# TimZaman/dotaclient

Hardware: NVIDIA H100
Metric: optimizer_steps_per_sec (higher is better)
Workload: dtype f32

## Files before the change

dotaclient_b200/csrc/dc_common.cuh:

```cuda
#pragma once
#include <cuda_runtime.h>
#include <stdint.h>
#include "dotaclient_b200.h"

void dc_set_error(const char *fmt, ...);

#define DC_REQUIRE(cond, code, ...)        \
    do {                                   \
        if (!(cond)) {                     \
            dc_set_error(__VA_ARGS__);     \
            return (code);                 \
        }                                  \
    } while (0)

#define DC_CUDA(call)                                                                      \
    do {                                                                                   \
        cudaError_t e__ = (call);                                                          \
        if (e__ != cudaSuccess) {                                                          \
            dc_set_error("%s failed at %s:%d: %s", #call, __FILE__, __LINE__,              \
                         cudaGetErrorString(e__));                                         \
            return (int)e__;                                                               \
        }                                                                                  \
    } while (0)

#define DC_LAUNCH_OK() DC_CUDA(cudaGetLastError())

static inline cudaStream_t dc_cu_stream(dc_stream_t s) { return reinterpret_cast<cudaStream_t>(s); }

int dc_sm_count();

int dc_gemm_tf32x3_splitk(const float *A, int lda, const float *B, int ldb, float *part, int64_t M, int N, int K, int ksplit,
                          bool first_call, cudaStream_t st);

int dc_unit_basic_reduce(const float *partial, int nblocks, float *dw_b, float *db_b, int accumulate, cudaStream_t st);

__device__ __forceinline__ float dc_sigmoid(float x) { return 1.0f / (1.0f + __expf(-x)); }
__device__ __forceinline__ float dc_tanh(float x) { return 1.0f - 2.0f / (__expf(2.0f * x) + 1.0f); }

__device__ __forceinline__ float2 dc_ffma2(float2 a, float2 b, float2 c) { return make_float2(fmaf(a.x, b.x, c.x), fmaf(a.y, b.y, c.y)); }

__device__ __forceinline__ uint32_t dc_smem_u32(const void *p) { return (uint32_t)__cvta_generic_to_shared(p); }
__device__ __forceinline__ float dc_tf32_rna(float v) { return __uint_as_float((__float_as_uint(v) + 0x1000u) & 0xffffe000u); }
__device__ __forceinline__ uint64_t dc_wgmma_desc(uint32_t smem_addr) {
    return (uint64_t)((smem_addr & 0x3FFFF) >> 4) | (1ull << 16) | ((uint64_t)(1024 >> 4) << 32) | (1ull << 62);
}
__device__ __forceinline__ void dc_wgmma_fence() { asm volatile("wgmma.fence.sync.aligned;" ::: "memory"); }
__device__ __forceinline__ void dc_wgmma_commit() { asm volatile("wgmma.commit_group.sync.aligned;" ::: "memory"); }
__device__ __forceinline__ void dc_wgmma_wait0() { asm volatile("wgmma.wait_group.sync.aligned 0;" ::: "memory"); }
__device__ __forceinline__ void dc_reg_fence(float &r) { asm volatile("" : "+f"(r)::"memory"); }
__device__ __forceinline__ void dc_mbar_init(uint64_t *bar, int count) {
    asm volatile("mbarrier.init.shared::cta.b64 [%0], %1;" ::"r"(dc_smem_u32(bar)), "r"(count));
}
__device__ __forceinline__ void dc_mbar_arrive(uint64_t *bar) {
    asm volatile("mbarrier.arrive.shared::cta.b64 _, [%0];" ::"r"(dc_smem_u32(bar)) : "memory");
}
__device__ __forceinline__ void dc_mbar_wait(uint64_t *bar, uint32_t parity) {
    uint32_t ok;
    do {
        asm volatile("{ .reg .pred p; mbarrier.try_wait.parity.shared::cta.b64 p, [%1], %2; selp.u32 %0, 1, 0, p; }"
                     : "=r"(ok)
                     : "r"(dc_smem_u32(bar)), "r"(parity)
                     : "memory");
    } while (!ok);
}

__device__ __forceinline__ float dc_warp_sum(float v) {
#pragma unroll
    for (int o = 16; o > 0; o >>= 1) v += __shfl_xor_sync(0xffffffffu, v, o);
    return v;
}
__device__ __forceinline__ double dc_warp_sum(double v) {
#pragma unroll
    for (int o = 16; o > 0; o >>= 1) v += __shfl_xor_sync(0xffffffffu, v, o);
    return v;
}
```

dotaclient_b200/csrc/gemm_tf32x3.cu:

```cuda
#include "dc_common.cuh"
#include "unit_basic.cuh"

namespace {

constexpr int BM = 128, BN = 128, BK = 32;
constexpr int kStages = 2;
constexpr int kTileBytes = BM * BK * 4;
constexpr int kStageBytes = 4 * kTileBytes;
constexpr int kProducerThreads = 128;
constexpr int kProducerGroups = kStages;
constexpr int kConsumerWarp0 = 4 * kProducerGroups;
constexpr int kConsumerThreads = 256;
constexpr int kThreads = kConsumerWarp0 * 32 + kConsumerThreads;
constexpr int kLdS = BN + 8;
constexpr int kDIn = kUnitFeatures;
constexpr size_t kOffStaging = (size_t)kStages * kStageBytes;
constexpr size_t kOffBars = kOffStaging + (size_t)BM * kLdS * 4;
constexpr size_t kSmemBytes = kOffBars + 128 + 1024 ;

#define DC_ACC8(b) "+f"(d[b]), "+f"(d[b + 1]), "+f"(d[b + 2]), "+f"(d[b + 3]), "+f"(d[b + 4]), "+f"(d[b + 5]), "+f"(d[b + 6]), "+f"(d[b + 7])
__device__ __forceinline__ void wgmma_m64n128k8(float (&d)[64], uint64_t desc_a, uint64_t desc_b) {
    asm volatile(
        "{\n\t.reg .pred p;\n\tsetp.ne.b32 p, %66, 0;\n\t"
        "wgmma.mma_async.sync.aligned.m64n128k8.f32.tf32.tf32 "
// ... 894 lines not shown
            const int t0 = (split + j * nsplit) * kRPC, tend = min(T, t0 + kRPC);
            const int s = j % kWgStages;
            dc_mbar_wait(&empty[s], ((j / kWgStages) & 1) ^ 1);
            unsigned char *st = ring + (size_t)s * kWgStageBytes;
            const uint32_t xs = dc_smem_u32(st + 2 * kTileBytes);
#pragma unroll
            for (int r = 0; r < BK / 4; ++r) {
                const int row = (t >> 5) + 4 * r;
                const bool ok = xc_in && t0 + row < tend;
                const size_t xr = kDevT && x_rows != nullptr && ok ? (size_t)__ldg(x_rows + t0 + row) : (size_t)(t0 + row);
                cp_async16(xs + (row * kWgLdX + 4 * xc) * 4, X + (ok ? xr * ldx + n0 + 4 * xc : 0), ok ? 16u : 0u);
            }
            cp_async_arrive(&full[s]);
            store_row_k(va, st, st + kTileBytes, t);
            asm volatile("fence.proxy.async.shared::cta;" ::: "memory");
            __syncwarp();
            if (lane == 0) dc_mbar_arrive(&full[s]);
        }
        colsum_s[g * 128 + t] = cs;
        asm volatile("cp.async.wait_all;" ::: "memory");
    } else {
        const int ct = threadIdx.x - kConsumerWarp0 * 32, wg = ct >> 7, w4 = (ct >> 5) & 3, q = lane & 3;
        const int rlo = 64 * wg + 16 * w4 + (lane >> 2);
        float d[64];
#pragma unroll
        for (int i = 0; i < 64; ++i) d[i] = 0.f;
        uint32_t ahi[2][4] = {}, alo[2][4] = {};
#pragma unroll
        for (int i = 0; i < 64; ++i) dc_reg_fence(d[i]);
        float *pt = part_w + ((size_t)split * tiles_mn + tile) * BM * BN + ct * 4;
        const auto flush = [&](bool add) {
            dc_wgmma_wait0();
#pragma unroll
            for (int k = 0; k < 64; ++k) dc_reg_fence(d[k]);
            if (add) {
#pragma unroll
                for (int m = 0; m < 16; ++m)
                    asm volatile("red.global.add.v4.f32 [%0], {%1, %2, %3, %4};" ::"l"(pt + m * kConsumerThreads * 4), "f"(d[4 * m]),
                                 "f"(d[4 * m + 1]), "f"(d[4 * m + 2]), "f"(d[4 * m + 3]) : "memory");
            } else {
#pragma unroll
                for (int m = 0; m < 16; ++m)
                    *reinterpret_cast<float4 *>(pt + m * kConsumerThreads * 4) = make_float4(d[4 * m], d[4 * m + 1], d[4 * m + 2], d[4 * m + 3]);
            }
#pragma unroll
            for (int k = 0; k < 64; ++k) d[k] = 0.f;
#pragma unroll
            for (int k = 0; k < 64; ++k) dc_reg_fence(d[k]);
        };
        int j = 0;
        do {
            const int j_end = min(my_chunks, j + kWgFlush);
            for (; j < j_end; ++j) {
                const int s = j % kWgStages;
                dc_mbar_wait(&full[s], (j / kWgStages) & 1);
                const uint32_t st = dc_smem_u32(ring + (size_t)s * kWgStageBytes);
                const uint32_t xk = st + 2 * kTileBytes + (q * kWgLdX + rlo) * 4;
                float v[16];
#pragma unroll
                for (int ks = 0; ks < BK / 8; ++ks) {
                    const uint32_t x8 = xk + 8 * ks * kWgLdX * 4;
                    v[4 * ks] = lds_f32(x8);
                    v[4 * ks + 1] = lds_f32(x8 + 8 * 4);
                    v[4 * ks + 2] = lds_f32(x8 + 4 * kWgLdX * 4);
                    v[4 * ks + 3] = lds_f32(x8 + (4 * kWgLdX + 8) * 4);
                }
                const uint64_t b_hi = dc_wgmma_desc(st), b_lo = dc_wgmma_desc(st + kTileBytes);
#pragma unroll
                for (int ks = 0; ks < BK / 8; ++ks) {
                    const int b = ks & 1;
#pragma unroll
                    for (int e = 0; e < 4; ++e) {
                        const float h = dc_tf32_rna(v[4 * ks + e]);
                        ahi[b][e] = __float_as_uint(h);
                        alo[b][e] = __float_as_uint(v[4 * ks + e] - h);
                    }
                    dc_wgmma_fence();
                    const uint64_t adv = (uint64_t)(ks * 2);
                    wgmma_m64n128k8_rs(d, ahi[b][0], ahi[b][1], ahi[b][2], ahi[b][3], b_lo + adv);
                    wgmma_m64n128k8_rs(d, alo[b][0], alo[b][1], alo[b][2], alo[b][3], b_hi + adv);
                    wgmma_m64n128k8_rs(d, ahi[b][0], ahi[b][1], ahi[b][2], ahi[b][3], b_hi + adv);
                    dc_wgmma_commit();
                    wgmma_wait1();
#pragma unroll
                    for (int e = 0; e < 4; ++e) asm volatile("" : "+r"(ahi[b ^ 1][e]), "+r"(alo[b ^ 1][e])::"memory");
                    if (ks == 0 && j > 0) {
                        __syncwarp();
                        if (lane == 0) dc_mbar_arrive(&empty[(j - 1) % kWgStages]);
                    }
                }
            }
            flush(j > kWgFlush);
        } while (j < my_chunks);
    }
    __syncthreads();
    if (part_b != nullptr && n0 == 0 && threadIdx.x < 128 && m0 + (int)threadIdx.x < No)
        part_b[(size_t)split * No + m0 + threadIdx.x] = colsum_s[threadIdx.x] + colsum_s[128 + threadIdx.x];
}

constexpr int kRedRows = 8;
__global__ void __launch_bounds__(32 * kRedRows) wgrad_reduce_kernel(const float *__restrict__ part_w, const float *__restrict__ part_b,
                                                                     int nsplit, int No, int Ni, float *__restrict__ dW, int ldw,
                                                                     float *__restrict__ db, int accumulate) {
    __shared__ float4 sh[kRedRows][32];
    const int x = threadIdx.x & 31, y = threadIdx.x >> 5;
    const int n_blocks = (Ni + BN - 1) / BN, tiles_mn = ((No + BM - 1) / BM) * n_blocks;
    const int total4 = tiles_mn * (BM * BN / 4), bias4 = db != nullptr ? No / 4 : 0;
    const int idx = blockIdx.x * 32 + x;
    const float *src = nullptr;
    size_t stride = 0;
    if (idx < total4) {
        src = part_w + (size_t)idx * 4;
        stride = (size_t)tiles_mn * BM * BN;
    } else if (idx < total4 + bias4) {
        src = part_b + (size_t)(idx - total4) * 4;
        stride = (size_t)No;
    }
    float4 acc = make_float4(0.f, 0.f, 0.f, 0.f);
    if (src != nullptr) {
#pragma unroll 4
        for (int s = y; s < nsplit; s += kRedRows) {
            const float4 v = __ldg(reinterpret_cast<const float4 *>(src + (size_t)s * stride));
            acc.x += v.x; acc.y += v.y; acc.z += v.z; acc.w += v.w;
        }
    }
    sh[y][x] = acc;
    __syncthreads();
    if (y == 0 && src != nullptr) {
        if (idx < total4) {
            const int tile = idx / (BM * BN / 4), r = idx % (BM * BN / 4), m = r / kConsumerThreads, ct = r % kConsumerThreads;
            const int o = (tile / n_blocks) * BM + 8 * m + 2 * (ct & 3);
            const int i = (tile % n_blocks) * BN + 64 * (ct >> 7) + 16 * ((ct >> 5) & 3) + ((ct & 31) >> 2);
            float *p[4];
            float v[4];
#pragma unroll
            for (int e = 0; e < 4; ++e) {
                const int oe = o + (e & 1), ie = i + 8 * (e >> 1);
                p[e] = oe < No && ie < Ni ? dW + (size_t)oe * ldw + ie : nullptr;
                v[e] = accumulate && p[e] != nullptr ? *p[e] : 0.f;
            }
#pragma unroll
            for (int r = 0; r < kRedRows; ++r) { v[0] += sh[r][x].x; v[1] += sh[r][x].y; v[2] += sh[r][x].z; v[3] += sh[r][x].w; }
#pragma unroll
            for (int e = 0; e < 4; ++e)
                if (p[e] != nullptr) *p[e] = v[e];
        } else {
            float *dst = db + (size_t)(idx - total4) * 4;
            float4 t = accumulate ? *reinterpret_cast<const float4 *>(dst) : make_float4(0.f, 0.f, 0.f, 0.f);
#pragma unroll
            for (int r = 0; r < kRedRows; ++r) { t.x += sh[r][x].x; t.y += sh[r][x].y; t.z += sh[r][x].z; t.w += sh[r][x].w; }
            *reinterpret_cast<float4 *>(dst) = t;
        }
    }
}

}

extern "C" int dc_gemm_tf32x3_supported(int64_t M, int N, int K) { return M > 0 && N > 0 && K > 0 && N % 32 == 0 && K % BK == 0; }

struct RowList {
    const int *count, *a_rows, *rows;
    float *C_rows;
};

template <int NU, bool kGenA = false, bool kDevM = false>
static int launch_ws(const float *A, int lda, const float *B, int ldb, const float *bias, float *C, int ldc, int M, int N,
                     int K, int relu, float *C_copy, uint8_t *argmax, cudaStream_t st, GenA gen = GenA{}, RowList rl = RowList{}) {
    const int tile_rows = NU == 5 ? 60 : kWsRows;
    const int n_blocks = (N + BN - 1) / BN, m_blocks = (M + tile_rows - 1) / tile_rows;
    int per_block = dc_sm_count() / n_blocks;
    if (per_block < 1) per_block = 1;
    if (per_block > m_blocks) per_block = m_blocks;
    const size_t smem = kGenA ? kWsGenSmemBytes : kWsSmemBytes;
    DC_CUDA(cudaFuncSetAttribute(gemm_ws_kernel<NU, kGenA, kDevM>, cudaFuncAttributeMaxDynamicSharedMemorySize, (int)smem));
    gemm_ws_kernel<NU, kGenA, kDevM><<<n_blocks * per_block, kWsThreads, smem, st>>>(A, lda, B, ldb, bias, C, ldc, M, N, K, relu, C_copy,
                                                                                    argmax, gen, rl.count, rl.a_rows, rl.rows, rl.C_rows);
    DC_LAUNCH_OK();
    return DC_OK;
}

static int gemm_check_shape(const float *A, int lda, const float *B, int ldb, const float *bias, const float *C, int ldc, int64_t M,
                            int N, int K, const char *who) {
    DC_REQUIRE(dc_gemm_tf32x3_supported(M, N, K) && M < (1ll << 31) - BM, DC_EUNSUPPORTED,
               "%s: need N %% 32 == 0 and K %% 32 == 0 (M=%lld N=%d K=%d)", who, (long long)M, N, K);
    DC_REQUIRE(lda >= K && ldb >= K && ldc >= N && lda % 4 == 0 && ldb % 4 == 0 && ldc % 4 == 0, DC_EINVAL,
               "%s: leading dimensions must be >= extent and multiples of 4 floats", who);
    DC_REQUIRE(((uintptr_t)A & 15) == 0 && ((uintptr_t)B & 15) == 0 && ((uintptr_t)C & 15) == 0 && (!bias || ((uintptr_t)bias & 15) == 0),
               DC_EINVAL, "%s: pointers must be 16-byte aligned", who);
    return DC_OK;
}

static int gemm_check(const float *A, int lda, const float *B, int ldb, const float *bias, const float *C, int ldc, int64_t M, int N,
                      int K, const char *who) {
    DC_REQUIRE(A && B && C, DC_EINVAL, "%s: null pointer", who);
    return gemm_check_shape(A, lda, B, ldb, bias, C, ldc, M, N, K, who);
}

template <bool kDevM>
static int gemm_launch(const float *A, int lda, const float *B, int ldb, const float *bias, float *C, int ldc, int64_t M, int N, int K,
                       int relu, RowList rl, cudaStream_t st) {
    if (K <= 4 * BK) return launch_ws<0, false, kDevM>(A, lda, B, ldb, bias, C, ldc, (int)M, N, K, relu, nullptr, nullptr, st, GenA{}, rl);
    const int tiles = (int)((M + BM - 1) / BM) * ((N + BN - 1) / BN);
    DC_CUDA(cudaFuncSetAttribute(gemm_tf32x3_kernel<kDevM>, cudaFuncAttributeMaxDynamicSharedMemorySize, (int)kSmemBytes));
    const int grid = tiles < dc_sm_count() ? tiles : dc_sm_count();
    gemm_tf32x3_kernel<kDevM><<<grid, kThreads, kSmemBytes, st>>>(A, lda, B, ldb, bias, C, ldc, (int)M, N, K, relu, 1, 0, rl.count,
                                                                  rl.a_rows, rl.rows, rl.C_rows);
    DC_LAUNCH_OK();
    return DC_OK;
}

extern "C" int dc_gemm_tf32x3(const float *A, int lda, const float *B, int ldb, const float *bias, float *C, int ldc,
                              int64_t M, int N, int K, int relu, dc_stream_t stream) {
    const int rc = gemm_check(A, lda, B, ldb, bias, C, ldc, M, N, K, "dc_gemm_tf32x3");
    if (rc != DC_OK) return rc;
    return gemm_launch<false>(A, lda, B, ldb, bias, C, ldc, M, N, K, relu, RowList{}, dc_cu_stream(stream));
}

extern "C" int dc_gemm_tf32x3_rows(const float *A, int lda, const float *B, int ldb, const float *bias, float *C, float *C_rows, int ldc,
                                   int64_t M, const int32_t *count, const int32_t *rows, int gather_a, int N, int K, int relu,
                                   dc_stream_t stream) {
    DC_REQUIRE(A && B && count && (C || C_rows) && (rows || (!gather_a && !C_rows)), DC_EINVAL, "dc_gemm_tf32x3_rows: null pointer");
    DC_REQUIRE(((uintptr_t)C_rows & 15) == 0, DC_EINVAL, "dc_gemm_tf32x3_rows: pointers must be 16-byte aligned");
    const int rc = gemm_check_shape(A, lda, B, ldb, bias, C, ldc, M, N, K, "dc_gemm_tf32x3_rows");
    if (rc != DC_OK) return rc;
    return gemm_launch<true>(A, lda, B, ldb, bias, C, ldc, M, N, K, relu, RowList{count, gather_a ? rows : nullptr, rows, C_rows},
                             dc_cu_stream(stream));
}

int dc_gemm_tf32x3_splitk(const float *A, int lda, const float *B, int ldb, float *part, int64_t M, int N, int K, int ksplit,
                          bool first_call, cudaStream_t st) {
    DC_REQUIRE(A && B && part && ksplit >= 1 && N % BN == 0 && K % (BK * ksplit) == 0 && M > 0, DC_EINVAL,
               "dc_gemm_tf32x3_splitk: bad arguments (M=%lld N=%d K=%d ksplit=%d)", (long long)M, N, K, ksplit);
    if (first_call)
        DC_CUDA(cudaFuncSetAttribute(gemm_tf32x3_kernel<false>, cudaFuncAttributeMaxDynamicSharedMemorySize, (int)kSmemBytes));
    const int tiles = (int)((M + BM - 1) / BM) * (N / BN) * ksplit;
    const int grid = tiles < dc_sm_count() ? tiles : dc_sm_count();
    gemm_tf32x3_kernel<false><<<grid, kThreads, kSmemBytes, st>>>(A, lda, B, ldb, nullptr, part, N, (int)M, N, K, 0, ksplit, (long long)M * N);
    DC_LAUNCH_OK();
    return DC_OK;
}

static int wgrad_tiles(int No, int Ni) { return ((No + BM - 1) / BM) * ((Ni + BN - 1) / BN); }

static int wgrad_splits(int No, int Ni) {
    const int tiles_mn = wgrad_tiles(No, Ni);
    const int n = dc_sm_count() / tiles_mn;
    return n < 1 ? 1 : n;
}

extern "C" size_t dc_gemm_wgrad_workspace_bytes(int No, int Ni) {
    if (No <= 0 || Ni <= 0 || No % 32 || Ni % 32) return 0;
    const int nsplit = wgrad_splits(No, Ni);
    return ((size_t)nsplit * wgrad_tiles(No, Ni) * BM * BN + (size_t)nsplit * No) * sizeof(float);
}

template <bool kDevT>
static int wgrad_launch(const float *dY, int ldy, const float *X, int ldx, int64_t T, const int *t_dev, const int *x_rows, int No, int Ni,
                        float *dW, int ldw, float *db, int accumulate, void *workspace, dc_stream_t stream, const char *who) {
    DC_REQUIRE(dY && X && dW && workspace && (!kDevT || t_dev), DC_EINVAL, "%s: null pointer", who);
    DC_REQUIRE(T > 0 && T < (1ll << 31) - BK && No > 0 && Ni > 0 && No % 32 == 0 && Ni % 32 == 0, DC_EUNSUPPORTED,
               "%s: need No %% 32 == 0 and Ni %% 32 == 0 (T=%lld No=%d Ni=%d)", who, (long long)T, No, Ni);
    DC_REQUIRE(ldy >= No && ldx >= Ni && ldw >= Ni && ldy % 4 == 0 && ldx % 4 == 0 && ldw % 4 == 0, DC_EINVAL,
               "%s: bad leading dimension", who);
    DC_REQUIRE(((uintptr_t)dY & 15) == 0 && ((uintptr_t)X & 15) == 0 && ((uintptr_t)dW & 15) == 0 && ((uintptr_t)workspace & 15) == 0 &&
                   ((uintptr_t)db & 15) == 0,
               DC_EINVAL, "%s: pointers must be 16-byte aligned", who);
    const int tiles_mn = wgrad_tiles(No, Ni), nsplit = wgrad_splits(No, Ni);
    float *part_w = reinterpret_cast<float *>(workspace);
    float *part_b = db ? part_w + (size_t)nsplit * tiles_mn * BM * BN : nullptr;
    cudaStream_t st = dc_cu_stream(stream);
    DC_CUDA(cudaFuncSetAttribute(gemm_wgrad_kernel<0, kDevT>, cudaFuncAttributeMaxDynamicSharedMemorySize, (int)kWgSmemBytes));
    gemm_wgrad_kernel<0, kDevT><<<tiles_mn * nsplit, kThreads, kWgSmemBytes, st>>>(dY, ldy, nullptr, nullptr, X, ldx, (int)T, No, Ni,
                                                                                   nsplit, part_w, part_b, t_dev, x_rows);
    DC_LAUNCH_OK();
    const int total4 = tiles_mn * (BM * BN / 4) + (db ? No / 4 : 0);
    wgrad_reduce_kernel<<<(total4 + 31) / 32, 32 * kRedRows, 0, st>>>(part_w, part_b, nsplit, No, Ni, dW, ldw, db, accumulate);
    DC_LAUNCH_OK();
    return DC_OK;
}

extern "C" int dc_gemm_wgrad_tf32x3(const float *dY, int ldy, const float *X, int ldx, int64_t T, int No, int Ni, float *dW,
                                    int ldw, float *db, int accumulate, void *workspace, dc_stream_t stream) {
    return wgrad_launch<false>(dY, ldy, X, ldx, T, nullptr, nullptr, No, Ni, dW, ldw, db, accumulate, workspace, stream,
                               "dc_gemm_wgrad_tf32x3");
}

extern "C" int dc_gemm_wgrad_tf32x3_rows(const float *dY, int ldy, const float *X, int ldx, const int32_t *x_rows, int64_t T,
                                         const int32_t *t_dev, int No, int Ni, float *dW, int ldw, float *db, int accumulate,
                                         void *workspace, dc_stream_t stream) {
    return wgrad_launch<true>(dY, ldy, X, ldx, T, t_dev, x_rows, No, Ni, dW, ldw, db, accumulate, workspace, stream,
                              "dc_gemm_wgrad_tf32x3_rows");
}

extern "C" int dc_gemm_unit_max(const float *basic, const float *w, const float *bias, float *xmax, float *xmax_copy, int ld_x,
                                uint8_t *argmax, int64_t n_tokens, int n_units, dc_stream_t stream) {
    DC_REQUIRE(basic && w && bias && xmax && argmax && n_tokens > 0, DC_EINVAL, "dc_gemm_unit_max: null pointer / empty input");
    DC_REQUIRE(n_units == 5 || n_units == 16, DC_EUNSUPPORTED, "dc_gemm_unit_max: n_units=%d (5 or 16; 1-unit groups are plain GEMMs)", n_units);
    DC_REQUIRE(ld_x >= BN && n_tokens * n_units < (1ll << 31) - BM, DC_EINVAL, "dc_gemm_unit_max: bad ld_x / size");
    DC_REQUIRE(((uintptr_t)basic & 15) == 0 && ((uintptr_t)w & 15) == 0, DC_EINVAL, "dc_gemm_unit_max: pointers must be 16-byte aligned");
    const int M = (int)(n_tokens * n_units);
    cudaStream_t st = dc_cu_stream(stream);
    if (n_units == 5) return launch_ws<5>(basic, BN, w, BN, bias, xmax, ld_x, M, BN, BN, 0, xmax_copy, argmax, st);
    return launch_ws<16>(basic, BN, w, BN, bias, xmax, ld_x, M, BN, BN, 0, xmax_copy, argmax, st);
}

extern "C" int dc_unit_embed_fwd_mask(const float *units, const float *w_b, const float *b_b, float *basic_out, uint32_t *mask_out,
                                      const float *w, const float *bias, float *xmax, float *xmax_copy, int ld_x, uint8_t *argmax,
                                      int64_t n_tokens, int n_units, dc_stream_t stream) {
    DC_REQUIRE(units && w_b && b_b && w && bias && xmax && n_tokens > 0, DC_EINVAL, "dc_unit_embed_fwd: null pointer / empty input");
    DC_REQUIRE(n_units == 1 || n_units == 5 || n_units == 16, DC_EUNSUPPORTED, "dc_unit_embed_fwd: n_units=%d (1, 5 or 16)", n_units);
    DC_REQUIRE(n_units == 1 ? (argmax == nullptr && xmax_copy == nullptr) : argmax != nullptr, DC_EINVAL,
               "dc_unit_embed_fwd: the arg-max (and the copy) go with the max-pool of n_units 5 and 16 only");
    DC_REQUIRE(ld_x >= BN && ld_x % 4 == 0 && n_tokens * n_units < (1ll << 31) - BM, DC_EINVAL, "dc_unit_embed_fwd: bad ld_x / size");
    DC_REQUIRE(((uintptr_t)units & 15) == 0 && ((uintptr_t)basic_out & 15) == 0 && ((uintptr_t)w & 15) == 0 && ((uintptr_t)bias & 15) == 0 &&
                   ((uintptr_t)xmax & 15) == 0 && ((uintptr_t)xmax_copy & 15) == 0 && ((uintptr_t)mask_out & 15) == 0,
               DC_EINVAL, "dc_unit_embed_fwd: units, basic_out, mask_out, w, bias, xmax, xmax_copy must be 16-byte aligned");
    const int M = (int)(n_tokens * n_units);
    const GenA gen{units, w_b, b_b, basic_out, mask_out};
    cudaStream_t st = dc_cu_stream(stream);
    if (n_units == 1) return launch_ws<0, true>(nullptr, BN, w, BN, bias, xmax, ld_x, M, BN, BN, 0, nullptr, nullptr, st, gen);
    if (n_units == 5) return launch_ws<5, true>(nullptr, BN, w, BN, bias, xmax, ld_x, M, BN, BN, 0, xmax_copy, argmax, st, gen);
    return launch_ws<16, true>(nullptr, BN, w, BN, bias, xmax, ld_x, M, BN, BN, 0, xmax_copy, argmax, st, gen);
}

extern "C" int dc_unit_embed_fwd(const float *units, const float *w_b, const float *b_b, float *basic_out, const float *w, const float *bias,
                                 float *xmax, float *xmax_copy, int ld_x, uint8_t *argmax, int64_t n_tokens, int n_units,
                                 dc_stream_t stream) {
    return dc_unit_embed_fwd_mask(units, w_b, b_b, basic_out, nullptr, w, bias, xmax, xmax_copy, ld_x, argmax, n_tokens, n_units, stream);
}

extern "C" int dc_unit_dgrad_fused_mask(const float *d_xmax, const float *d_xmax2, int ld_dx, const uint8_t *argmax, const float *dlogits,
                                        int ld_dl, const float *att, const float *w_t, const float *units, const uint32_t *mask,
                                        const float *w_b, const float *b_b, int64_t n_tokens, int n_units, float *dw_b, float *db_b,
                                        int accumulate, void *workspace, dc_stream_t stream) {
    DC_REQUIRE(w_t && units && w_b && b_b && dw_b && db_b && workspace && n_tokens > 0, DC_EINVAL, "dc_unit_dgrad_fused: null pointer / empty input");
    DC_REQUIRE(n_units == 1 || n_units == 5 || n_units == 16, DC_EUNSUPPORTED, "dc_unit_dgrad_fused: n_units=%d (1, 5 or 16)", n_units);
    DC_REQUIRE((d_xmax == nullptr && d_xmax2 == nullptr) || (d_xmax != nullptr && ld_dx >= BN && ld_dx % 4 == 0), DC_EINVAL,
               "dc_unit_dgrad_fused: bad d_xmax / ld_dx");
    DC_REQUIRE(d_xmax == nullptr || n_units == 1 || argmax != nullptr, DC_EINVAL, "dc_unit_dgrad_fused: routing needs the arg-max");
    DC_REQUIRE((dlogits == nullptr) == (att == nullptr) && (dlogits == nullptr || ld_dl >= n_units), DC_EINVAL,
               "dc_unit_dgrad_fused: dlogits and att come together");
    DC_REQUIRE(n_tokens * n_units < (1ll << 31) - BM, DC_EINVAL, "dc_unit_dgrad_fused: too many rows");
    DC_REQUIRE(((uintptr_t)d_xmax & 15) == 0 && ((uintptr_t)d_xmax2 & 15) == 0 && ((uintptr_t)argmax & 3) == 0 && ((uintptr_t)att & 15) == 0 &&
                   ((uintptr_t)w_t & 15) == 0 && ((uintptr_t)units & 15) == 0 && ((uintptr_t)mask & 15) == 0 && ((uintptr_t)workspace & 15) == 0,
               DC_EINVAL, "dc_unit_dgrad_fused: d_xmax, att, w_t, units, mask must be 16-byte aligned (arg-max 4-byte)");
    const int n_tok = (int)n_tokens;
    const int tile_rows = BM - BM % n_units;
    int grid = (int)((n_tokens * n_units + tile_rows - 1) / tile_rows);
    if (grid > dc_sm_count()) grid = dc_sm_count();
    float *partial = reinterpret_cast<float *>(workspace);
    cudaStream_t st = dc_cu_stream(stream);
#define DC_LAUNCH_DGRAD(NU, MASK)                                                                                                    \
    do {                                                                                                                              \
        DC_CUDA(cudaFuncSetAttribute(unit_dgrad_kernel<NU, MASK>, cudaFuncAttributeMaxDynamicSharedMemorySize, (int)kDgSmemBytes)); \
        unit_dgrad_kernel<NU, MASK><<<grid, kThreads, kDgSmemBytes, st>>>(d_xmax, d_xmax2, ld_dx, argmax, dlogits, ld_dl, att, w_t,  \
                                                                          units, mask, w_b, b_b, n_tok, partial);                     \
    } while (0)
    if (mask != nullptr) {
        if (n_units == 1) DC_LAUNCH_DGRAD(1, true);
        else if (n_units == 5) DC_LAUNCH_DGRAD(5, true);
        else DC_LAUNCH_DGRAD(16, true);
    } else {
        if (n_units == 1) DC_LAUNCH_DGRAD(1, false);
        else if (n_units == 5) DC_LAUNCH_DGRAD(5, false);
        else DC_LAUNCH_DGRAD(16, false);
    }
#undef DC_LAUNCH_DGRAD
    DC_LAUNCH_OK();
    return dc_unit_basic_reduce(partial, grid, dw_b, db_b, accumulate, st);
}

extern "C" int dc_unit_dgrad_fused(const float *d_xmax, const float *d_xmax2, int ld_dx, const uint8_t *argmax, const float *dlogits,
                                   int ld_dl, const float *att, const float *w_t, const float *units, const float *w_b,
                                   const float *b_b, int64_t n_tokens, int n_units, float *dw_b, float *db_b, int accumulate,
                                   void *workspace, dc_stream_t stream) {
    return dc_unit_dgrad_fused_mask(d_xmax, d_xmax2, ld_dx, argmax, dlogits, ld_dl, att, w_t, units, nullptr, w_b, b_b, n_tokens, n_units,
                                    dw_b, db_b, accumulate, workspace, stream);
}

extern "C" int dc_unit_wgrad_routed(const float *d_xmax, const float *d_xmax2, int ld_dx, const uint8_t *argmax, const float *basic,
                                    int64_t n_tokens, int n_units, float *dW, float *db, void *workspace, dc_stream_t stream) {
    DC_REQUIRE(d_xmax && argmax && basic && dW && db && workspace && n_tokens > 0, DC_EINVAL, "dc_unit_wgrad_routed: null pointer / empty input");
    DC_REQUIRE(n_units == 5 || n_units == 16, DC_EUNSUPPORTED, "dc_unit_wgrad_routed: n_units=%d (5 or 16; a 1-unit group is dc_gemm_wgrad_tf32x3)", n_units);
    DC_REQUIRE(ld_dx >= BM && n_tokens * n_units < (1ll << 31) - BK, DC_EINVAL, "dc_unit_wgrad_routed: bad ld_dx / size");
    DC_REQUIRE(((uintptr_t)basic & 15) == 0 && ((uintptr_t)dW & 15) == 0 && ((uintptr_t)db & 15) == 0 && ((uintptr_t)workspace & 15) == 0,
               DC_EINVAL, "dc_unit_wgrad_routed: pointers must be 16-byte aligned");
    const int No = BM, Ni = BN, nsplit = wgrad_splits(No, Ni);
    const int T = (int)(n_tokens * n_units);
    float *part_w = reinterpret_cast<float *>(workspace);
    float *part_b = part_w + (size_t)nsplit * No * Ni;
    cudaStream_t st = dc_cu_stream(stream);
    if (n_units == 5) {
        DC_CUDA(cudaFuncSetAttribute(gemm_wgrad_kernel<5>, cudaFuncAttributeMaxDynamicSharedMemorySize, (int)kWgSmemBytes));
        gemm_wgrad_kernel<5><<<nsplit, kThreads, kWgSmemBytes, st>>>(d_xmax, ld_dx, d_xmax2, argmax, basic, BN, T, No, Ni, nsplit,
                                                                                part_w, part_b);
    } else {
        DC_CUDA(cudaFuncSetAttribute(gemm_wgrad_kernel<16>, cudaFuncAttributeMaxDynamicSharedMemorySize, (int)kWgSmemBytes));
        gemm_wgrad_kernel<16><<<nsplit, kThreads, kWgSmemBytes, st>>>(d_xmax, ld_dx, d_xmax2, argmax, basic, BN, T, No, Ni, nsplit,
                                                                                 part_w, part_b);
    }
    DC_LAUNCH_OK();
    wgrad_reduce_kernel<<<(BM * BN / 4 + No / 4 + 31) / 32, 32 * kRedRows, 0, st>>>(part_w, part_b, nsplit, No, Ni, dW, Ni, db, 0);
    DC_LAUNCH_OK();
    return DC_OK;
}
```

dotaclient_b200/csrc/rnn_resident.cuh:

```cuda
#pragma once
#include "rnn_cell.cuh"

namespace dc_rnn {

constexpr int kH = 128;
constexpr int kStages = 4;

__device__ __forceinline__ void mbar_expect_tx(uint64_t *bar, uint32_t bytes) {
    asm volatile("mbarrier.arrive.expect_tx.shared::cta.b64 _, [%0], %1;" ::"r"(dc_smem_u32(bar)), "r"(bytes) : "memory");
}
__device__ __forceinline__ void bulk_g2s(void *dst, const void *src, uint32_t bytes, uint64_t *bar) {
    asm volatile("cp.async.bulk.shared::cluster.global.mbarrier::complete_tx::bytes [%0], [%1], %2, [%3];" ::"r"(
                     dc_smem_u32(dst)),
                 "l"(src), "r"(bytes), "r"(dc_smem_u32(bar))
                 : "memory");
}

template <int NT, int NOUT>
struct Tiling {
    static constexpr int NCG = NOUT / 4;
    static constexpr int NMS = NT / NCG;
    static constexpr int M = NMS * 32;
};

template <int NT, int NOUT>
__device__ __forceinline__ void load_weights(const float *__restrict__ A, float2 (&wr)[8][4], float4 *w_s) {
    using T = Tiling<NT, NOUT>;
    const int cg = threadIdx.x % T::NCG, ms = threadIdx.x / T::NCG;
#pragma unroll
    for (int j = 0; j < 8; ++j) {
        const float4 r0 = __ldg(reinterpret_cast<const float4 *>(A + (size_t)(ms * 32 + 2 * j) * NOUT) + cg);
        const float4 r1 = __ldg(reinterpret_cast<const float4 *>(A + (size_t)(ms * 32 + 2 * j + 1) * NOUT) + cg);
        wr[j][0] = make_float2(r0.x, r1.x); wr[j][1] = make_float2(r0.y, r1.y);
        wr[j][2] = make_float2(r0.z, r1.z); wr[j][3] = make_float2(r0.w, r1.w);
    }
#pragma unroll
    for (int j = 0; j < 8; ++j) {
        const float4 r0 = __ldg(reinterpret_cast<const float4 *>(A + (size_t)(ms * 32 + 16 + 2 * j) * NOUT) + cg);
        const float4 r1 = __ldg(reinterpret_cast<const float4 *>(A + (size_t)(ms * 32 + 17 + 2 * j) * NOUT) + cg);
        w_s[((ms * 8 + j) * 2 + 0) * T::NCG + cg] = make_float4(r0.x, r1.x, r0.y, r1.y);
        w_s[((ms * 8 + j) * 2 + 1) * T::NCG + cg] = make_float4(r0.z, r1.z, r0.w, r1.w);
    }
}

template <int NT, int NOUT, int BT>
__device__ __forceinline__ void matvec_partial(const float2 (&wr)[8][4], const float4 *w_s, const float *in_s, float *part_s) {
    using T = Tiling<NT, NOUT>;
    const int cg = threadIdx.x % T::NCG, ms = threadIdx.x / T::NCG;
    float2 acc[BT][4];
#pragma unroll
    for (int b = 0; b < BT; ++b)
#pragma unroll
        for (int c = 0; c < 4; ++c) acc[b][c] = make_float2(0.f, 0.f);
    const float *in0 = in_s + ms * 32;
#pragma unroll
    for (int j = 0; j < 8; j += 2) {
        float4 hv[BT];
#pragma unroll
        for (int b = 0; b < BT; ++b) hv[b] = *reinterpret_cast<const float4 *>(in0 + b * T::M + 2 * j);
#pragma unroll
        for (int b = 0; b < BT; ++b) {
            const float2 h0 = make_float2(hv[b].x, hv[b].y), h1 = make_float2(hv[b].z, hv[b].w);
#pragma unroll
            for (int c = 0; c < 4; ++c) {
                acc[b][c] = dc_ffma2(h0, wr[j][c], acc[b][c]);
                acc[b][c] = dc_ffma2(h1, wr[j + 1][c], acc[b][c]);
            }
        }
    }
    const float4 *wp = w_s + (ms * 16) * T::NCG + cg;
#pragma unroll
    for (int j = 0; j < 8; j += 2) {
        float4 hv[BT];
#pragma unroll
        for (int b = 0; b < BT; ++b) hv[b] = *reinterpret_cast<const float4 *>(in0 + b * T::M + 16 + 2 * j);
#pragma unroll
        for (int p = 0; p < 2; ++p) {
            const float4 wa = wp[((j + p) * 2 + 0) * T::NCG];
            const float4 wb = wp[((j + p) * 2 + 1) * T::NCG];
            const float2 w0 = make_float2(wa.x, wa.y), w1 = make_float2(wa.z, wa.w);
            const float2 w2 = make_float2(wb.x, wb.y), w3 = make_float2(wb.z, wb.w);
#pragma unroll
            for (int b = 0; b < BT; ++b) {
                const float2 h = p == 0 ? make_float2(hv[b].x, hv[b].y) : make_float2(hv[b].z, hv[b].w);
                acc[b][0] = dc_ffma2(h, w0, acc[b][0]);
                acc[b][1] = dc_ffma2(h, w1, acc[b][1]);
                acc[b][2] = dc_ffma2(h, w2, acc[b][2]);
                acc[b][3] = dc_ffma2(h, w3, acc[b][3]);
            }
        }
    }
#pragma unroll
    for (int b = 0; b < BT; ++b)
        *reinterpret_cast<float4 *>(part_s + ((ms * BT + b) * NOUT) + cg * 4) =
            make_float4(acc[b][0].x + acc[b][0].y, acc[b][1].x + acc[b][1].y, acc[b][2].x + acc[b][2].y, acc[b][3].x + acc[b][3].y);
}

template <int G, int BT>
struct FwdSmem {
    static constexpr int NT = G * kH;
    static constexpr int GH = G * kH;
    static constexpr size_t w_bytes = (size_t)NT * 16 * sizeof(float4);
    static constexpr size_t in_bytes = (size_t)BT * kH * 4;
    static constexpr size_t part_bytes = (size_t)4 * BT * GH * 4;
    static constexpr size_t stage_bytes = (size_t)BT * GH * 4;
    static constexpr size_t total = w_bytes + in_bytes + part_bytes + kStages * stage_bytes + kStages * 8 + 16;
};

template <int G, int BT, bool kReset = false>
__global__ void __launch_bounds__(G *kH, 1) fwd_resident_kernel(float *__restrict__ gates, const float *__restrict__ wT,
                                                                 const float *__restrict__ b_hh, float *__restrict__ ybuf,
                                                                 float *__restrict__ cbuf, int B, int S, Reset rs) {
    using SM = FwdSmem<G, BT>;
    constexpr int NT = SM::NT, GH = SM::GH, H = kH;
    static_assert(BT * kH <= G * kH, "one gate thread per (sequence, unit) pair");
    extern __shared__ __align__(128) unsigned char smem_raw[];
    float4 *w_s = reinterpret_cast<float4 *>(smem_raw);
    float *in_s = reinterpret_cast<float *>(smem_raw + SM::w_bytes);
    float *part_s = reinterpret_cast<float *>(smem_raw + SM::w_bytes + SM::in_bytes);
    float *stage_s = reinterpret_cast<float *>(smem_raw + SM::w_bytes + SM::in_bytes + SM::part_bytes);
    uint64_t *bars = reinterpret_cast<uint64_t *>(smem_raw + SM::w_bytes + SM::in_bytes + SM::part_bytes + kStages * SM::stage_bytes);

    const int tid = threadIdx.x;
    const int b0 = blockIdx.x * BT;
    const int nb = min(BT, B - b0);
    const uint32_t tile_bytes = (uint32_t)nb * GH * 4;

    float2 wr[8][4];
    load_weights<NT, GH>(wT, wr, w_s);
    if (tid == 0) {
        for (int s = 0; s < kStages; ++s) dc_mbar_init(&bars[s], 1);
        asm volatile("fence.mbarrier_init.release.cluster;" ::: "memory");
    }
    const bool unit = tid < BT * H;
    const int ub = tid / H, uu = tid % H;
    const bool live = unit && ub < nb;
    float c_reg = 0.f, bias[G];
    if (unit) {
        in_s[ub * H + uu] = live ? ybuf[(size_t)(b0 + ub) * H + uu] : 0.f;
        if (G == 4 && live) c_reg = cbuf[(size_t)(b0 + ub) * H + uu];
#pragma unroll
        for (int g = 0; g < G; ++g) bias[g] = b_hh[g * H + uu];
    }
    __syncthreads();
    if (tid == 0) {
        for (int s = 0; s < kStages && s < S; ++s) {
            mbar_expect_tx(&bars[s], tile_bytes);
            bulk_g2s(stage_s + (size_t)s * BT * GH, gates + ((size_t)s * B + b0) * GH, tile_bytes, &bars[s]);
        }
    }
    for (int t = 0; t < S; ++t) {
        int k = -1;
        if constexpr (kReset) k = live ? __ldg(rs.slot + (size_t)t * B + b0 + ub) : -1;
        matvec_partial<NT, GH, BT>(wr, w_s, in_s, part_s);
        __syncthreads();
        const int st = t % kStages;
        if (unit) {
            dc_mbar_wait(&bars[st], (t / kStages) & 1);
            if (live) {
                const float *gi = stage_s + (size_t)st * BT * GH + ub * GH;
                float pre[G];
#pragma unroll
                for (int g = 0; g < G; ++g) {
                    float a = bias[g];
#pragma unroll
                    for (int ms = 0; ms < 4; ++ms) a += part_s[(ms * BT + ub) * GH + g * H + uu];
                    pre[g] = a;
                }
                float prev = G == 3 ? in_s[ub * H + uu] : c_reg;
                if (kReset && k >= 0) {
                    const size_t r = (size_t)k * B + b0 + ub;
#pragma unroll
                    for (int g = 0; g < G; ++g) pre[g] = rs.pre[r * GH + g * H + uu];
                    prev = rs.prev[r * H + uu];
                }
                const size_t tok = (size_t)t * B + b0 + ub;
                float *gout = gates + tok * GH;
                float act[G], aux;
                const float hnew = cell_fwd<G, false>([&](int g) { return gi[g * H + uu]; }, [&](int g) { return pre[g]; },
                                               prev, act, aux);
                if (G == 4) c_reg = aux;
#pragma unroll
                for (int g = 0; g < G; ++g) gout[g * H + uu] = act[g];
                cbuf[(tok + B) * H + uu] = aux;
                ybuf[(tok + B) * H + uu] = hnew;
                in_s[ub * H + uu] = hnew;
            }
        }
        __syncthreads();
        if (tid == 0 && t + kStages < S) {
            mbar_expect_tx(&bars[st], tile_bytes);
            bulk_g2s(stage_s + (size_t)st * BT * GH, gates + ((size_t)(t + kStages) * B + b0) * GH, tile_bytes, &bars[st]);
        }
    }
}

template <int G, int BT>
struct BwdSmem {
    static constexpr int NT = G * kH;
    static constexpr int GH = G * kH;
    static constexpr int NMS = NT / (kH / 4);
    static constexpr size_t w_bytes = (size_t)NT * 16 * sizeof(float4);
    static constexpr size_t in_bytes = (size_t)BT * GH * 4;
    static constexpr size_t part_bytes = (size_t)NMS * BT * kH * 4;
    static constexpr size_t stage_floats = (size_t)BT * (GH + 3 * kH);
    static constexpr size_t total = w_bytes + in_bytes + part_bytes + kStages * stage_floats * 4 + kStages * 8 + 16;
};

template <int G, int BT, bool kReset = false>
__global__ void __launch_bounds__(G *kH, 1) bwd_resident_kernel(float *__restrict__ gates, const float *__restrict__ w,
                                                                 const float *__restrict__ ybuf, float *__restrict__ cbuf,
                                                                 const float *__restrict__ dy, const float *__restrict__ dhn,
                                                                 const float *__restrict__ dcn, float *__restrict__ dh0,
                                                                 float *__restrict__ dc0, int B, int S, Reset rs) {
    using SM = BwdSmem<G, BT>;
    constexpr int NT = SM::NT, GH = SM::GH, H = kH, NMS = SM::NMS;
    static_assert(BT * kH <= G * kH, "one gate thread per (sequence, unit) pair");
    extern __shared__ __align__(128) unsigned char smem_raw[];
    float4 *w_s = reinterpret_cast<float4 *>(smem_raw);
    float *in_s = reinterpret_cast<float *>(smem_raw + SM::w_bytes);
    float *part_s = reinterpret_cast<float *>(smem_raw + SM::w_bytes + SM::in_bytes);
    float *stage_s = reinterpret_cast<float *>(smem_raw + SM::w_bytes + SM::in_bytes + SM::part_bytes);
    uint64_t *bars = reinterpret_cast<uint64_t *>(smem_raw + SM::w_bytes + SM::in_bytes + SM::part_bytes + kStages * SM::stage_floats * 4);

    const int tid = threadIdx.x;
    const int b0 = blockIdx.x * BT;
    const int nb = min(BT, B - b0);
    const uint32_t gate_bytes = (uint32_t)nb * GH * 4, row_bytes = (uint32_t)nb * H * 4;

    float2 wr[8][4];
    load_weights<NT, H>(w, wr, w_s);
    if (tid == 0) {
        for (int s = 0; s < kStages; ++s) dc_mbar_init(&bars[s], 1);
        asm volatile("fence.mbarrier_init.release.cluster;" ::: "memory");
    }
    const bool unit = tid < BT * H;
    const int ub = tid / H, uu = tid % H;
    const bool live = unit && ub < nb;
    float dh_carry = 0.f;
    float dc_carry = 0.f;
    float c_cur = 0.f;
    if (live) {
        if (dhn) dh_carry = dhn[(size_t)(b0 + ub) * H + uu];
        if (G == 4) {
            if (dcn) dc_carry = dcn[(size_t)(b0 + ub) * H + uu];
            c_cur = cbuf[((size_t)S * B + b0 + ub) * H + uu];
        }
    }
    for (int i = tid; i < NMS * BT * H; i += NT) part_s[i] = 0.f;
    for (int i = tid; i < BT * GH; i += NT) in_s[i] = 0.f;
    __syncthreads();

    auto issue = [&](int t, int st) {
        float *dst = stage_s + (size_t)st * SM::stage_floats;
        const size_t tok = (size_t)t * B + b0;
        const uint32_t total = gate_bytes + row_bytes * (G == 3 ? 3u : 2u);
        mbar_expect_tx(&bars[st], total);
        bulk_g2s(dst, gates + tok * GH, gate_bytes, &bars[st]);
        bulk_g2s(dst + BT * GH, dy + tok * H, row_bytes, &bars[st]);
        if (G == 4) {
            bulk_g2s(dst + BT * (GH + H), cbuf + tok * H, row_bytes, &bars[st]);
        } else {
            bulk_g2s(dst + BT * (GH + H), cbuf + (tok + B) * H, row_bytes, &bars[st]);
            bulk_g2s(dst + BT * (GH + 2 * H), ybuf + tok * H, row_bytes, &bars[st]);
        }
    };
    if (tid == 0)
        for (int s = 0; s < kStages && s < S; ++s) issue(S - 1 - s, s);

    for (int it = 0; it < S; ++it) {
        const int t = S - 1 - it;
        const int st = it % kStages;
        if (unit) {
            int k = -1;
            if constexpr (kReset) k = live ? __ldg(rs.slot + (size_t)t * B + b0 + ub) : -1;
            dc_mbar_wait(&bars[st], (it / kStages) & 1);
            if (live) {
                const float *sg = stage_s + (size_t)st * SM::stage_floats;
                const float *g = sg + ub * GH;
                float dh = sg[BT * GH + ub * H + uu] + dh_carry;
#pragma unroll
                for (int ms = 0; ms < NMS; ++ms) dh += part_s[(ms * BT + ub) * H + uu];
                const size_t tok = (size_t)t * B + b0 + ub;
                float *gout = gates + tok * GH;
                float *dg = in_s + ub * GH;
                auto act = [&](int q) { return g[q * H + uu]; };
                const float aux1 = sg[BT * (GH + H) + ub * H + uu];
                float dgi[G], dgh[G];
                if constexpr (kReset) {
                    float prev = G == 3 ? sg[BT * (GH + 2 * H) + ub * H + uu] : aux1;
                    if (k >= 0) prev = rs.prev[((size_t)k * B + b0 + ub) * H + uu];
                    dh_carry = cell_bwd<G>(act, G == 3 ? aux1 : c_cur, prev, dh, dc_carry, dgi, dgh);
                } else {
                    if (G == 3) dh_carry = cell_bwd<G>(act, aux1, sg[BT * (GH + 2 * H) + ub * H + uu], dh, dc_carry, dgi, dgh);
                    else dh_carry = cell_bwd<G>(act, c_cur, aux1, dh, dc_carry, dgi, dgh);
                }
#pragma unroll
                for (int q = 0; q < G; ++q) gout[q * H + uu] = dgi[q];
                if (G == 3) cbuf[(tok + B) * H + uu] = dgh[2];
                if (kReset && k >= 0) {
                    dh_carry = 0.f;
                    dc_carry = 0.f;
#pragma unroll
                    for (int q = 0; q < G; ++q) dgh[q] = 0.f;
                }
#pragma unroll
                for (int q = 0; q < G; ++q) dg[q * H + uu] = dgh[q];
                if (G == 4) c_cur = aux1;
            }
        }
        __syncthreads();
        if (tid == 0 && it + kStages < S) issue(S - 1 - (it + kStages), st);
        matvec_partial<NT, H, BT>(wr, w_s, in_s, part_s);
        __syncthreads();
    }
    if (live) {
        float dh = dh_carry;
#pragma unroll
        for (int ms = 0; ms < NMS; ++ms) dh += part_s[(ms * BT + ub) * H + uu];
        if (dh0) dh0[(size_t)(b0 + ub) * H + uu] = dh;
        if (G == 4 && dc0) dc0[(size_t)(b0 + ub) * H + uu] = dc_carry;
    }
}

inline bool resident_supported(int H) { return H == kH; }

template <int G, int BT, bool kReset>
int launch_fwd_t(float *gates, const float *wT, const float *b_hh, float *ybuf, float *cbuf, int B, int S, Reset rs, cudaStream_t st) {
    const size_t smem = FwdSmem<G, BT>::total;
    DC_CUDA(cudaFuncSetAttribute(fwd_resident_kernel<G, BT, kReset>, cudaFuncAttributeMaxDynamicSharedMemorySize, (int)smem));
    fwd_resident_kernel<G, BT, kReset><<<(B + BT - 1) / BT, G * kH, smem, st>>>(gates, wT, b_hh, ybuf, cbuf, B, S, rs);
    DC_LAUNCH_OK();
    return DC_OK;
}
template <int G, int BT, bool kReset>
int launch_bwd_t(float *gates, const float *w, const float *ybuf, float *cbuf, const float *dy, const float *dhn,
                 const float *dcn, float *dh0, float *dc0, int B, int S, Reset rs, cudaStream_t st) {
    const size_t smem = BwdSmem<G, BT>::total;
    DC_CUDA(cudaFuncSetAttribute(bwd_resident_kernel<G, BT, kReset>, cudaFuncAttributeMaxDynamicSharedMemorySize, (int)smem));
    bwd_resident_kernel<G, BT, kReset><<<(B + BT - 1) / BT, G * kH, smem, st>>>(gates, w, ybuf, cbuf, dy, dhn, dcn, dh0, dc0, B, S, rs);
    DC_LAUNCH_OK();
    return DC_OK;
}

inline bool small_tile(int B) { return (B + 1) / 2 <= dc_sm_count(); }

template <bool kReset>
inline int launch_fwd_resident(int cell, float *gates, const float *w_hh, const float *b_hh, float *ybuf, float *cbuf, int B,
                               int S, void *workspace, Reset rs, cudaStream_t st) {
    float *wT = reinterpret_cast<float *>(workspace);
    int rc = launch_transpose(w_hh, wT, (cell == DC_CELL_GRU ? 3 : 4) * kH, kH, st);
    if (rc) return rc;
    if (cell == DC_CELL_GRU)
        return small_tile(B) ? launch_fwd_t<3, 2, kReset>(gates, wT, b_hh, ybuf, cbuf, B, S, rs, st)
                             : launch_fwd_t<3, 3, kReset>(gates, wT, b_hh, ybuf, cbuf, B, S, rs, st);
    return small_tile(B) ? launch_fwd_t<4, 2, kReset>(gates, wT, b_hh, ybuf, cbuf, B, S, rs, st)
                         : launch_fwd_t<4, 4, kReset>(gates, wT, b_hh, ybuf, cbuf, B, S, rs, st);
}
template <bool kReset>
inline int launch_bwd_resident(int cell, float *gates, const float *w, const float *ybuf, float *cbuf, const float *dy,
                               const float *dhn, const float *dcn, float *dh0, float *dc0, int B, int S, Reset rs, cudaStream_t st) {
    if (cell == DC_CELL_GRU)
        return small_tile(B) ? launch_bwd_t<3, 2, kReset>(gates, w, ybuf, cbuf, dy, dhn, dcn, dh0, dc0, B, S, rs, st)
                             : launch_bwd_t<3, 3, kReset>(gates, w, ybuf, cbuf, dy, dhn, dcn, dh0, dc0, B, S, rs, st);
    return small_tile(B) ? launch_bwd_t<4, 2, kReset>(gates, w, ybuf, cbuf, dy, dhn, dcn, dh0, dc0, B, S, rs, st)
                         : launch_bwd_t<4, 4, kReset>(gates, w, ybuf, cbuf, dy, dhn, dcn, dh0, dc0, B, S, rs, st);
}

}
```

Before: 91.06.

## Replace 16-unit wgrad GEMM with argmax-routed gather-FMA kernel

Measured after the change: 92.86, median of 6. 2.0% higher.

```diff
diff --git a/dotaclient_b200/csrc/dc_common.cuh b/dotaclient_b200/csrc/dc_common.cuh
--- a/dotaclient_b200/csrc/dc_common.cuh
+++ b/dotaclient_b200/csrc/dc_common.cuh
@@ -54,6 +54,15 @@
 __device__ __forceinline__ void dc_mbar_arrive(uint64_t *bar) {
     asm volatile("mbarrier.arrive.shared::cta.b64 _, [%0];" ::"r"(dc_smem_u32(bar)) : "memory");
 }
+__device__ __forceinline__ void dc_mbar_expect_tx(uint64_t *bar, uint32_t bytes) {
+    asm volatile("mbarrier.arrive.expect_tx.shared::cta.b64 _, [%0], %1;" ::"r"(dc_smem_u32(bar)), "r"(bytes) : "memory");
+}
+__device__ __forceinline__ void dc_bulk_g2s(void *dst, const void *src, uint32_t bytes, uint64_t *bar) {
+    asm volatile("cp.async.bulk.shared::cluster.global.mbarrier::complete_tx::bytes [%0], [%1], %2, [%3];" ::"r"(
+                     dc_smem_u32(dst)),
+                 "l"(src), "r"(bytes), "r"(dc_smem_u32(bar))
+                 : "memory");
+}
 __device__ __forceinline__ void dc_mbar_wait(uint64_t *bar, uint32_t parity) {
     uint32_t ok;
     do {
diff --git a/dotaclient_b200/csrc/gemm_tf32x3.cu b/dotaclient_b200/csrc/gemm_tf32x3.cu
--- a/dotaclient_b200/csrc/gemm_tf32x3.cu
+++ b/dotaclient_b200/csrc/gemm_tf32x3.cu
@@ -1070,6 +1070,124 @@
             *reinterpret_cast<float4 *>(dst) = t;
         }
     }
+}
+
+constexpr int kAmTok = 8;
+constexpr int kAmStages = 3;
+constexpr int kAmWarps = 8;
+constexpr int kAmThreads = 32 * (kAmWarps + 1);
+constexpr int kAmTokBytes = 16 * BN * 4;
+constexpr int kAmOffG = kAmTok * kAmTokBytes;
+constexpr int kAmOffArg = kAmOffG + kAmTok * BM * 4;
+constexpr int kAmStageBytes = kAmOffArg + kAmTok * BM;
+constexpr size_t kAmOffBars = (size_t)kAmStages * kAmStageBytes;
+constexpr size_t kAmSmemBytes = kAmOffBars + 2 * kAmStages * 8;
+constexpr int kAmFlush = kWgFlush * BK;
+static_assert(kAmStageBytes % 16 == 0 && kAmFlush % kAmTok == 0, "stage layout");
+static_assert(kAmSmemBytes <= 227 * 1024, "arg-max weight gradient exceeds the shared-memory opt-in");
+
+__global__ void __maxnreg__(128) unit_wgrad_argmax_kernel(const float *__restrict__ dx, const float *__restrict__ dx2,
+                                                                          int ld_dx, const uint8_t *__restrict__ argmax,
+                                                                          const float *__restrict__ basic, int n_tok,
+                                                                          float *__restrict__ part_w, float *__restrict__ part_b) {
+    extern __shared__ __align__(16) unsigned char sm[];
+    uint64_t *full = reinterpret_cast<uint64_t *>(sm + kAmOffBars), *empty = full + kAmStages;
+    const int warp = threadIdx.x >> 5, lane = threadIdx.x & 31;
+    const int tok0 = (int)((long long)n_tok * blockIdx.x / gridDim.x), tok1 = (int)((long long)n_tok * (blockIdx.x + 1) / gridDim.x);
+    const int n_stages = (tok1 - tok0 + kAmTok - 1) / kAmTok;
+    if (threadIdx.x == 0) {
+        for (int s = 0; s < kAmStages; ++s) { dc_mbar_init(&full[s], 2); dc_mbar_init(&empty[s], kAmWarps); }
+        asm volatile("fence.mbarrier_init.release.cluster;" ::: "memory");
+    }
+    __syncthreads();
+
+    if (warp == kAmWarps) {
+        for (int j = 0; j < n_stages; ++j) {
+            const int s = j % kAmStages, t0 = tok0 + j * kAmTok, nt = min(kAmTok, tok1 - t0);
+            float gv[kAmTok][4];
+            uint32_t av[kAmTok][4];
+#pragma unroll
+            for (int k = 0; k < kAmTok; ++k) {
+                const size_t n = (size_t)(k < nt ? t0 + k : t0);
+#pragma unroll
+                for (int e = 0; e < 4; ++e) {
+                    const int c = lane + 32 * e;
+                    gv[k][e] = __ldg(dx + n * ld_dx + c);
+                    if (dx2 != nullptr) gv[k][e] += __ldg(dx2 + n * ld_dx + c);
+                    av[k][e] = __ldg(argmax + n * BM + c);
+                }
+            }
+            dc_mbar_wait(&empty[s], ((j / kAmStages) & 1) ^ 1);
+            unsigned char *st = sm + (size_t)s * kAmStageBytes;
+            if (lane == 0) {
+                dc_mbar_expect_tx(&full[s], (uint32_t)nt * kAmTokBytes);
+                dc_bulk_g2s(st, basic + (size_t)t0 * 16 * BN, (uint32_t)nt * kAmTokBytes, &full[s]);
+            }
+            float *gs = reinterpret_cast<float *>(st + kAmOffG);
+            uint8_t *as = st + kAmOffArg;
+#pragma unroll
+            for (int k = 0; k < kAmTok; ++k)
+#pragma unroll
+                for (int e = 0; e < 4; ++e) {
+                    gs[k * BM + lane + 32 * e] = gv[k][e];
+                    as[k * BM + lane + 32 * e] = (uint8_t)av[k][e];
+                }
+            __syncwarp();
+            if (lane == 0) dc_mbar_arrive(&full[s]);
+        }
+        return;
+    }
+
+    const int c0 = 16 * warp;
+    float acc[16][4];
+#pragma unroll
+    for (int c = 0; c < 16; ++c) acc[c][0] = acc[c][1] = acc[c][2] = acc[c][3] = 0.f;
+    float bs = 0.f, bc = 0.f;
+    float *pw = part_w + (size_t)blockIdx.x * BM * BN + (size_t)(2 * warp) * kConsumerThreads * 4 +
+                (128 * (lane >> 4) + 32 * ((lane >> 2) & 3) + 16 * (lane & 1)) * 4 + 2 * ((lane >> 1) & 1);
+    const auto flush = [&](bool add) {
+#pragma unroll
+        for (int c = 0; c < 16; ++c)
+#pragma unroll
+            for (int e = 0; e < 4; ++e) {
+                float *p = pw + (c >> 3) * kConsumerThreads * 4 + (4 * e + ((c >> 1) & 3)) * 4 + (c & 1);
+                *p = add ? *p + acc[c][e] : acc[c][e];
+                acc[c][e] = 0.f;
+            }
+    };
+    for (int j = 0; j < n_stages; ++j) {
+        const int s = j % kAmStages, nt = min(kAmTok, tok1 - tok0 - j * kAmTok);
+        dc_mbar_wait(&full[s], (j / kAmStages) & 1);
+        const unsigned char *st = sm + (size_t)s * kAmStageBytes;
+#pragma unroll 1
+        for (int k = 0; k < nt; ++k) {
+            const float4 *g4 = reinterpret_cast<const float4 *>(st + kAmOffG + (k * BM + c0) * 4);
+            const float4 ga = g4[0], gb = g4[1], gc = g4[2], gd = g4[3];
+            const float g[16] = {ga.x, ga.y, ga.z, ga.w, gb.x, gb.y, gb.z, gb.w, gc.x, gc.y, gc.z, gc.w, gd.x, gd.y, gd.z, gd.w};
+            const uint4 a4 = *reinterpret_cast<const uint4 *>(st + kAmOffArg + k * BM + c0);
+            const uint32_t a[4] = {a4.x, a4.y, a4.z, a4.w};
+            const unsigned char *rows = st + k * kAmTokBytes + lane * 16;
+#pragma unroll
+            for (int c = 0; c < 16; ++c) {
+                const uint32_t u = (a[c >> 2] >> (8 * (c & 3))) & 15u;
+                const float4 x = *reinterpret_cast<const float4 *>(rows + u * (BN * 4));
+                acc[c][0] = fmaf(g[c], x.x, acc[c][0]);
+                acc[c][1] = fmaf(g[c], x.y, acc[c][1]);
+                acc[c][2] = fmaf(g[c], x.z, acc[c][2]);
+                acc[c][3] = fmaf(g[c], x.w, acc[c][3]);
+            }
+            if (lane < 16) {
+                const float y = reinterpret_cast<const float *>(st + kAmOffG)[k * BM + c0 + lane] - bc, t = bs + y;
+                bc = (t - bs) - y;
+                bs = t;
+            }
+        }
+        __syncwarp();
+        if (lane == 0) dc_mbar_arrive(&empty[s]);
+        if ((j + 1) % (kAmFlush / kAmTok) == 0 && j + 1 < n_stages) flush(j + 1 > kAmFlush / kAmTok);
+    }
+    flush(n_stages > kAmFlush / kAmTok);
+    if (lane < 16) part_b[(size_t)blockIdx.x * BM + c0 + lane] = bs;
 }
 
 }
@@ -1313,9 +1431,9 @@
         gemm_wgrad_kernel<5><<<nsplit, kThreads, kWgSmemBytes, st>>>(d_xmax, ld_dx, d_xmax2, argmax, basic, BN, T, No, Ni, nsplit,
                                                                                 part_w, part_b);
     } else {
-        DC_CUDA(cudaFuncSetAttribute(gemm_wgrad_kernel<16>, cudaFuncAttributeMaxDynamicSharedMemorySize, (int)kWgSmemBytes));
-        gemm_wgrad_kernel<16><<<nsplit, kThreads, kWgSmemBytes, st>>>(d_xmax, ld_dx, d_xmax2, argmax, basic, BN, T, No, Ni, nsplit,
-                                                                                 part_w, part_b);
+        DC_CUDA(cudaFuncSetAttribute(unit_wgrad_argmax_kernel, cudaFuncAttributeMaxDynamicSharedMemorySize, (int)kAmSmemBytes));
+        unit_wgrad_argmax_kernel<<<nsplit, kAmThreads, kAmSmemBytes, st>>>(d_xmax, d_xmax2, ld_dx, argmax, basic, (int)n_tokens,
+                                                                           part_w, part_b);
     }
     DC_LAUNCH_OK();
     wgrad_reduce_kernel<<<(BM * BN / 4 + No / 4 + 31) / 32, 32 * kRedRows, 0, st>>>(part_w, part_b, nsplit, No, Ni, dW, Ni, db, 0);
diff --git a/dotaclient_b200/csrc/rnn_resident.cuh b/dotaclient_b200/csrc/rnn_resident.cuh
--- a/dotaclient_b200/csrc/rnn_resident.cuh
+++ b/dotaclient_b200/csrc/rnn_resident.cuh
@@ -5,16 +5,6 @@
 
 constexpr int kH = 128;
 constexpr int kStages = 4;
-
-__device__ __forceinline__ void mbar_expect_tx(uint64_t *bar, uint32_t bytes) {
-    asm volatile("mbarrier.arrive.expect_tx.shared::cta.b64 _, [%0], %1;" ::"r"(dc_smem_u32(bar)), "r"(bytes) : "memory");
-}
-__device__ __forceinline__ void bulk_g2s(void *dst, const void *src, uint32_t bytes, uint64_t *bar) {
-    asm volatile("cp.async.bulk.shared::cluster.global.mbarrier::complete_tx::bytes [%0], [%1], %2, [%3];" ::"r"(
-                     dc_smem_u32(dst)),
-                 "l"(src), "r"(bytes), "r"(dc_smem_u32(bar))
-                 : "memory");
-}
 
 template <int NT, int NOUT>
 struct Tiling {
@@ -145,8 +135,8 @@
     __syncthreads();
     if (tid == 0) {
         for (int s = 0; s < kStages && s < S; ++s) {
-            mbar_expect_tx(&bars[s], tile_bytes);
-            bulk_g2s(stage_s + (size_t)s * BT * GH, gates + ((size_t)s * B + b0) * GH, tile_bytes, &bars[s]);
+            dc_mbar_expect_tx(&bars[s], tile_bytes);
+            dc_bulk_g2s(stage_s + (size_t)s * BT * GH, gates + ((size_t)s * B + b0) * GH, tile_bytes, &bars[s]);
         }
     }
     for (int t = 0; t < S; ++t) {
@@ -189,8 +179,8 @@
         }
         __syncthreads();
         if (tid == 0 && t + kStages < S) {
-            mbar_expect_tx(&bars[st], tile_bytes);
-            bulk_g2s(stage_s + (size_t)st * BT * GH, gates + ((size_t)(t + kStages) * B + b0) * GH, tile_bytes, &bars[st]);
+            dc_mbar_expect_tx(&bars[st], tile_bytes);
+            dc_bulk_g2s(stage_s + (size_t)st * BT * GH, gates + ((size_t)(t + kStages) * B + b0) * GH, tile_bytes, &bars[st]);
         }
     }
 }
@@ -255,14 +245,14 @@
         float *dst = stage_s + (size_t)st * SM::stage_floats;
         const size_t tok = (size_t)t * B + b0;
         const uint32_t total = gate_bytes + row_bytes * (G == 3 ? 3u : 2u);
-        mbar_expect_tx(&bars[st], total);
-        bulk_g2s(dst, gates + tok * GH, gate_bytes, &bars[st]);
-        bulk_g2s(dst + BT * GH, dy + tok * H, row_bytes, &bars[st]);
+        dc_mbar_expect_tx(&bars[st], total);
+        dc_bulk_g2s(dst, gates + tok * GH, gate_bytes, &bars[st]);
+        dc_bulk_g2s(dst + BT * GH, dy + tok * H, row_bytes, &bars[st]);
         if (G == 4) {
-            bulk_g2s(dst + BT * (GH + H), cbuf + tok * H, row_bytes, &bars[st]);
+            dc_bulk_g2s(dst + BT * (GH + H), cbuf + tok * H, row_bytes, &bars[st]);
         } else {
-            bulk_g2s(dst + BT * (GH + H), cbuf + (tok + B) * H, row_bytes, &bars[st]);
-            bulk_g2s(dst + BT * (GH + 2 * H), ybuf + tok * H, row_bytes, &bars[st]);
+            dc_bulk_g2s(dst + BT * (GH + H), cbuf + (tok + B) * H, row_bytes, &bars[st]);
+            dc_bulk_g2s(dst + BT * (GH + 2 * H), ybuf + tok * H, row_bytes, &bars[st]);
         }
     };
     if (tid == 0)
```
